# Hawkeye-FineGrained/Hawkeye

Hardware: NVIDIA H100
Metric: 448x448 images/sec, BCNN VGG-16 train step (fwd+CE+bwd+grad all-reduce+SGD), device-timed, max over ranks (higher is better)
Workload: dtype tf32 (fp32 storage, fp32 accumulate)

## Files before the change

### hawkeye_b200/csrc/conv.cu

```cuda
#include <stdlib.h>

#include "common.cuh"
#include "host.h"
#include "gemm.h"
#include "../../include/hawkeye_b200.h"

namespace hk {

__global__ void pack_weights_kernel(const float* __restrict__ W, float* __restrict__ Wf, float* __restrict__ Wd,
                                    int Cout, int Cin, int round) {
  const size_t n = (size_t)Cout * Cin * 9;
  for (size_t i = blockIdx.x * (size_t)blockDim.x + threadIdx.x; i < n; i += (size_t)gridDim.x * blockDim.x) {
    const int t = i % 9;
    const int ci = (i / 9) % Cin;
    const int co = i / ((size_t)9 * Cin);
    const float v = round ? tf32_round(W[i]) : W[i];
    if (Wf) Wf[((size_t)t * Cout + co) * Cin + ci] = v;
    if (Wd) Wd[((size_t)(8 - t) * Cin + ci) * Cout + co] = v;
  }
}
__global__ void unpack_wgrad_kernel(const float* __restrict__ dWp, float* __restrict__ dW, int Cout, int Cin, int accumulate) {
  const size_t n = (size_t)Cout * Cin * 9;
  for (size_t i = blockIdx.x * (size_t)blockDim.x + threadIdx.x; i < n; i += (size_t)gridDim.x * blockDim.x) {
    const int t = i % 9;
    const int ci = (i / 9) % Cin;
    const int co = i / ((size_t)9 * Cin);
    const float v = dWp[((size_t)t * Cin + ci) * Cout + co];
    dW[i] = accumulate ? dW[i] + v : v;
  }
}

struct ConvArgs {
  float* Y;
  const float* bias;
  const float* mask;
  int N, H, W, Cin, Cout;
  int TW, TH, TN;
  int tiles_w, tiles_h, tiles_n;
  int relu;
  int stride;
  const float* addend;
  int no_round;
  float* P;
  unsigned char* code;
  int pool_nchw;
};

__device__ __forceinline__ void epi_pool_store(const ConvArgs& a, const float* v, int TW, int w, int h, int n, int co,
                                               bool valid) {
  const bool writer = valid && !(w & 1) && !(h & 1);
  const int Ho = a.H >> 1, Wo = a.W >> 1;
  const size_t pp = ((size_t)n * Ho + (h >> 1)) * Wo + (w >> 1);
  float m[32];
  unsigned char cd[32];
#pragma unroll
  for (int j = 0; j < 32; ++j) {
    const float v0 = v[j];
    const float v1 = __shfl_xor_sync(0xffffffffu, v0, 1);
    const float v2 = __shfl_xor_sync(0xffffffffu, v0, TW);
    const float v3 = __shfl_xor_sync(0xffffffffu, v0, TW | 1);
    float mm = v0;
    unsigned char k = 0;
    if (v1 > mm) { mm = v1; k = 1; }
    if (v2 > mm) { mm = v2; k = 2; }
    if (v3 > mm) { mm = v3; k = 3; }
    m[j] = mm;
    cd[j] = k | (mm > 0.f ? 4 : 0);
  }
  if (!writer) return;
  if (a.code) {
    uint32_t pk[8];
#pragma unroll
    for (int j = 0; j < 8; ++j)
      pk[j] = (uint32_t)cd[4 * j] | ((uint32_t)cd[4 * j + 1] << 8) | ((uint32_t)cd[4 * j + 2] << 16) | ((uint32_t)cd[4 * j + 3] << 24);
    uint4* cp = reinterpret_cast<uint4*>(a.code + pp * a.Cout + co);
    cp[0] = make_uint4(pk[0], pk[1], pk[2], pk[3]);
    cp[1] = make_uint4(pk[4], pk[5], pk[6], pk[7]);
  }
  if (!a.pool_nchw) {
    float4* dst = reinterpret_cast<float4*>(a.P + pp * a.Cout + co);
#pragma unroll
    for (int j = 0; j < 8; ++j) dst[j] = make_float4(m[4 * j], m[4 * j + 1], m[4 * j + 2], m[4 * j + 3]);
  } else {
    const size_t hw = (size_t)Ho * Wo;
    float* dst = a.P + ((size_t)n * a.Cout + co) * hw + (size_t)(h >> 1) * Wo + (w >> 1);
#pragma unroll
    for (int j = 0; j < 32; ++j) dst[(size_t)j * hw] = m[j];
  }
}

constexpr int CONV_THREADS = 384;

template <int BN>
struct ConvCfg {
  static constexpr int STAGES = 4;
  static constexpr int A_BYTES = 128 * 128;
  static constexpr int B_BYTES = BN * 128;
  static constexpr int STAGE_BYTES = A_BYTES + B_BYTES;
  static constexpr int ACC_TILE = 2 * 128 * 33 * 4;
  static constexpr int SMEM = STAGES * STAGE_BYTES + 1024 + 256 + ACC_TILE;
};

template <bool POOLED = false>
__device__ __forceinline__ void epi_chunk(const ConvArgs& a, float (&v)[32], int w, int h, int n, size_t pix, int co,
                                          bool valid) {
  if (valid && co < a.Cout) {
    if (!POOLED && a.addend) {
      const float4* ad = reinterpret_cast<const float4*>(a.addend + pix * a.Cout + co);
#pragma unroll
      for (int j = 0; j < 8; ++j) {
        const float4 t = ad[j];
// ... 114 lines not shown
        const int tap = kb / nchunk, ck = kb - tap * nchunk;
        const int kh = tap / 3, kw = tap - kh * 3;
        mbar_wait(&empty[s], ph ^ 1);
        mbar_expect_tx(&full[s], Cfg::STAGE_BYTES);
        tma_load_4d(sA + s * Cfg::A_BYTES, &tmX, &full[s], ck * 32, w0 * a.stride + kw - 1, h0 * a.stride + kh - 1, n0);
        tma_load_3d(sB + s * Cfg::B_BYTES, &tmW, &full[s], ck * 32, co0, tap);
      }
    }
  } else {
    regs_alloc<224>();
    const int ct = threadIdx.x - 128;
    const int wg = ct >> 7;
    float acc[NACC];
    for (int kb = 0; kb < nk; ++kb) {
      const int s = kb % Cfg::STAGES;
      const uint32_t ph = (kb / Cfg::STAGES) & 1;
      mbar_wait(&full[s], ph);
      const uint64_t a_base = make_sdesc(smem_u32(sA + s * Cfg::A_BYTES + wg * 64 * 128));
      const uint64_t b_base = make_sdesc(smem_u32(sB + s * Cfg::B_BYTES));
      wgmma_fence();
#pragma unroll
      for (int ks = 0; ks < 4; ++ks) wgmma_tf32(acc, a_base + ks * 2, b_base + ks * 2, (kb | ks) != 0);
      wgmma_commit();
      wgmma_wait<1>();
      wgmma_keep(acc);
      if (kb > 0 && (ct & 127) == 0) mbar_arrive(&empty[(kb - 1) % Cfg::STAGES]);
    }
    wgmma_wait<0>();
    wgmma_keep(acc);
    conv_epilogue<BN>(a, acc, acc_tile, w0, h0, n0, co0, ct);
  }
}

static void pick_tile(int W, int H, int N, int target, int* TW, int* TH, int* TN) {
  int tw = 1;
  while (tw * 2 <= 16 && W % (tw * 2) == 0 && tw * 2 <= target) tw *= 2;
  int th = 1;
  while (th * 2 * tw <= target && H % (th * 2) == 0) th *= 2;
  int tn = target / (tw * th);
  *TW = tw; *TH = th; *TN = tn;
  (void)N;
}

static int make_act_map(CUtensorMap* tm, const float* X, int N, int H, int W, int C, int TW, int TH, int TN,
                        int stride = 1) {
  uint64_t dims[4] = {(uint64_t)C, (uint64_t)W, (uint64_t)H, (uint64_t)N};
  uint64_t strides[3] = {(uint64_t)C * 4, (uint64_t)W * C * 4, (uint64_t)H * W * C * 4};
  uint32_t box[4] = {32, (uint32_t)(TW * stride), (uint32_t)(TH * stride), (uint32_t)TN};
  uint32_t estr[4] = {1, (uint32_t)stride, (uint32_t)stride, 1};
  return make_tmap(tm, X, 4, dims, strides, box, stride > 1 ? estr : nullptr);
}

template <int BN>
static int launch_conv(const CUtensorMap& tmX, const CUtensorMap& tmW, const ConvArgs& a, cudaStream_t stream) {
  using Cfg = ConvCfg<BN>;
  if (int r = allow_dynamic_smem<conv3x3_igemm_kernel<BN>>(Cfg::SMEM, BN == 64 ? "conv<64>" : "conv<128>")) return r;
  dim3 grid(a.tiles_w * a.tiles_h * a.tiles_n, (a.Cout + BN - 1) / BN);
  conv3x3_igemm_kernel<BN><<<grid, CONV_THREADS, Cfg::SMEM, stream>>>(tmX, tmW, a);
  HK_LAUNCH_CHECK("conv3x3_igemm_kernel");
  return 0;
}

constexpr int CONV_V2_THREADS = 512;

enum { EPI_MAP = 0, EPI_UNPOOL = 1, EPI_FIRST_WGRAD = 2 };
constexpr int FW_HALO = 3 * 10 * 18;
constexpr int FW_HALO_BYTES = 2 * FW_HALO * 4;
struct FirstWgradArgs {
  const float* img;
  float* part;
};

__device__ __forceinline__ void mma_m16n8k8_tf32(float (&d)[4], const uint32_t (&a)[4], uint32_t b0, uint32_t b1) {
  asm volatile("mma.sync.aligned.m16n8k8.row.col.f32.tf32.tf32.f32 {%0, %1, %2, %3}, {%4, %5, %6, %7}, {%8, %9}, "
               "{%0, %1, %2, %3};\n"
               : "+f"(d[0]), "+f"(d[1]), "+f"(d[2]), "+f"(d[3])
               : "r"(a[0]), "r"(a[1]), "r"(a[2]), "r"(a[3]), "r"(b0), "r"(b1));
}

template <int BN, bool RESIDENT>
struct ConvV2Cfg {
  static constexpr int A_BYTES = 160 * 128;
  static constexpr int B_TILE = BN * 128;
  static constexpr int STAGE_BYTES = A_BYTES + (RESIDENT ? 0 : 3 * B_TILE);
  static constexpr int STAGES = RESIDENT ? 2 : (BN == 64 ? 3 : 2);
  static constexpr int WRES_BYTES = RESIDENT ? 18 * B_TILE : 0;
  static constexpr int PIECES = STAGES == 2 && !RESIDENT ? 3 : 1;
  static constexpr int STG_LD = BN + 8;
  static constexpr int STG_BYTES = 128 * STG_LD * 4;
  static constexpr int SMEM = STAGES * STAGE_BYTES + WRES_BYTES + 1024 + 256 + STG_BYTES;
};

template <int BN, bool RESIDENT, int TW, int EPI>
__global__ void __launch_bounds__(CONV_V2_THREADS, 1)
conv3x3_igemm_v2_kernel(const __grid_constant__ CUtensorMap tmX, const __grid_constant__ CUtensorMap tmW, ConvArgs a,
                        int n_ntiles, int total_tiles, FirstWgradArgs fw) {
  using Cfg = ConvV2Cfg<BN, RESIDENT>;
  static_assert(EPI != EPI_FIRST_WGRAD || (BN == 64 && RESIDENT && TW == 16), "conv1_1 weight gradient: 64 -> 64, 16 x 8");
  constexpr int NACC = BN / 2;
  constexpr int TN = 16 / TW;
  constexpr int WG_ROWS = TW == 16 ? 64 : 80;
  extern __shared__ uint8_t smem_raw[];
  uint8_t* smem = reinterpret_cast<uint8_t*>((reinterpret_cast<uintptr_t>(smem_raw) + 1023) & ~uintptr_t(1023));
  uint8_t* stages = smem;
  uint8_t* wres = smem + Cfg::STAGES * Cfg::STAGE_BYTES;
  uint64_t* full = reinterpret_cast<uint64_t*>(wres + Cfg::WRES_BYTES);
  uint64_t* empty = full + Cfg::STAGES * Cfg::PIECES;
  uint64_t* wbar = empty + Cfg::STAGES;
  uint64_t* stg_full = wbar + 1;
  uint64_t* stg_empty = wbar + 2;
  float* stg = reinterpret_cast<float*>(wres + Cfg::WRES_BYTES + 256);

  const int warp = threadIdx.x >> 5;
  const int nchunk = a.Cin / 32;
  const int nkb = nchunk * 3;

  if (threadIdx.x == 0) {
    tma_prefetch_desc(&tmX);
    tma_prefetch_desc(&tmW);
    for (int s = 0; s < Cfg::STAGES; ++s) mbar_init(&empty[s], 2);
    for (int i = 0; i < Cfg::STAGES * Cfg::PIECES; ++i) mbar_init(&full[i], 1);
    mbar_init(wbar, 1);
    mbar_init(stg_full, 256);
    mbar_init(stg_empty, 128);
    fence_barrier_init();
  }
  __syncthreads();

  if (warp >= 12 && EPI == EPI_MAP && a.P) {
    const int r = threadIdx.x - 384;
    int j = 0;
    for (int t = blockIdx.x; t < total_tiles; t += gridDim.x, ++j) {
      int pt = t / n_ntiles;
      const int co0 = (t - pt * n_ntiles) * BN;
      const int tw = pt % a.tiles_w; pt /= a.tiles_w;
      const int th = pt % a.tiles_h; pt /= a.tiles_h;
      mbar_wait(stg_full, j & 1);
      const int w = tw * TW + (r & (TW - 1)), h = th * 8 + ((r / TW) & 7), n = pt * TN + r / (TW * 8);
      const bool valid = TN == 1 || n < a.N;
      const size_t pix = ((size_t)n * a.H + h) * a.W + w;
#pragma unroll 1
      for (int c = 0; c < BN / 32; ++c) {
        float v[32];
        const float4* src = reinterpret_cast<const float4*>(stg + r * Cfg::STG_LD + c * 32);
#pragma unroll
        for (int k = 0; k < 8; ++k) {
          const float4 q = src[k];
          v[4 * k] = q.x; v[4 * k + 1] = q.y; v[4 * k + 2] = q.z; v[4 * k + 3] = q.w;
        }
        if (c == BN / 32 - 1) mbar_arrive(stg_empty);
        epi_chunk<true>(a, v, w, h, n, pix, co0 + c * 32, valid);
      }
    }
  } else if (warp >= 12) {
    const int e = threadIdx.x - 384;
    const int ew = e >> 5, sub = (e >> 3) & 3, u4 = (e & 7) * 4;
    const int p0 = ew * 32 + sub;
    const int eoff0 = (TW == 16 ? (p0 >> 4) * a.W + (p0 & 15) : ((p0 >> 6) * a.H + ((p0 >> 3) & 7)) * a.W + (p0 & 7)) * a.Cout + u4;
    const int erow = a.W * a.Cout, e4 = 4 * a.Cout;
    auto eoff = [&](int k) { return eoff0 + (k / (TW / 4)) * erow + (k % (TW / 4)) * e4; };
    const float* srow = stg + (ew * 32 + sub) * Cfg::STG_LD + u4;
    auto tile_org = [&](int t, size_t& org, int& co0) {
      co0 = (t % n_ntiles) * BN;
      int pt = t / n_ntiles;
      const int tw = pt % a.tiles_w; pt /= a.tiles_w;
      const int th = pt % a.tiles_h; pt /= a.tiles_h;
      org = (((size_t)pt * TN * a.H + th * 8) * a.W + tw * TW) * a.Cout;
      return pt * TN + (TW == 16 ? 0 : ew >> 1) < a.N;
    };
    auto tile_pos = [&](int t, int& tw, int& th, int& tn) {
      int pt = t / n_ntiles;
      tw = pt % a.tiles_w; pt /= a.tiles_w;
      th = pt % a.tiles_h; tn = pt / a.tiles_h;
    };
    const int frow = 2 * a.W * a.Cout;
    const int uoff0 = (TW == 16 ? 2 * (p0 >> 4) * frow + 2 * (p0 & 15) * a.Cout
                                : ((p0 >> 6) * 2 * a.H + 2 * ((p0 >> 3) & 7)) * frow + 2 * (p0 & 7) * a.Cout) + u4;
    auto uoff = [&](int k) { return uoff0 + (k / (TW / 4)) * 2 * frow + (k % (TW / 4)) * 8 * a.Cout; };
    float* halo = stg + 128 * Cfg::STG_LD;
    float dacc[4][4] = {};
    const int lane = e & 31, g = lane >> 2, tq = lane & 3;
    int hoff[4];
#pragma unroll
    for (int nt = 0; nt < 4; ++nt) {
      const int jj = 8 * nt + g;
      hoff[nt] = jj < 27 ? (jj / 9) * 180 + (jj % 9 / 3) * 18 + jj % 3 : 0;
    }
    int co0 = 0, j = 0;
    size_t org = 0;
    for (int t = blockIdx.x; t < total_tiles; t += gridDim.x, ++j) {
      const bool valid = tile_org(t, org, co0);
      if constexpr (EPI == EPI_FIRST_WGRAD) {
        int tw, th, tn;
        tile_pos(t, tw, th, tn);
        float* hb = halo + (j & 1) * FW_HALO;
        for (int i = e; i < FW_HALO; i += 128) {
          const int ci = i / 180, hh = th * 8 - 1 + i / 18 % 10, ww = tw * 16 - 1 + i % 18;
          hb[i] = hh >= 0 && hh < a.H && ww >= 0 && ww < a.W
                      ? tf32_round(__ldg(fw.img + (((size_t)tn * 3 + ci) * a.H + hh) * a.W + ww)) : 0.f;
        }
      }
      mbar_wait(stg_full, j & 1);
#pragma unroll
      for (int c = 0; c < BN / 32; ++c) {
// ... 21 lines not shown
#pragma unroll
            for (int k = 0; k < 8; ++k) mk[k] = __ldcs(reinterpret_cast<const float4*>(a.mask + org + co + eoff(k)));
#pragma unroll
            for (int k = 0; k < 8; ++k) {
              v[k].x = mk[k].x > 0.f ? v[k].x : 0.f; v[k].y = mk[k].y > 0.f ? v[k].y : 0.f;
              v[k].z = mk[k].z > 0.f ? v[k].z : 0.f; v[k].w = mk[k].w > 0.f ? v[k].w : 0.f;
            }
          }
          if constexpr (EPI == EPI_MAP) {
#pragma unroll
            for (int k = 0; k < 8; ++k)
              __stcs(reinterpret_cast<float4*>(a.Y + org + co + eoff(k)),
                     make_float4(tf32_round(v[k].x), tf32_round(v[k].y), tf32_round(v[k].z), tf32_round(v[k].w)));
          } else if constexpr (EPI == EPI_UNPOOL) {
            int tw, th, tn;
            tile_pos(t, tw, th, tn);
            float* dst = a.Y + (((size_t)tn * TN * 2 * a.H + th * 16) * 2 * a.W + tw * 2 * TW) * a.Cout + co;
            uint32_t cd[8];
#pragma unroll
            for (int k = 0; k < 8; ++k) cd[k] = __ldcs(reinterpret_cast<const unsigned int*>(a.code + org + co + eoff(k)));
#pragma unroll
            for (int k = 0; k < 8; ++k) {
              const float4 q = make_float4((cd[k] & 4u) ? tf32_round(v[k].x) : 0.f, (cd[k] & (4u << 8)) ? tf32_round(v[k].y) : 0.f,
                                           (cd[k] & (4u << 16)) ? tf32_round(v[k].z) : 0.f,
                                           (cd[k] & (4u << 24)) ? tf32_round(v[k].w) : 0.f);
              float* o = dst + uoff(k);
#pragma unroll
              for (int pos = 0; pos < 4; ++pos)
                __stcs(reinterpret_cast<float4*>(o + (pos >> 1) * frow + (pos & 1) * a.Cout),
                       make_float4((cd[k] & 3u) == (uint32_t)pos ? q.x : 0.f, (cd[k] >> 8 & 3u) == (uint32_t)pos ? q.y : 0.f,
                                   (cd[k] >> 16 & 3u) == (uint32_t)pos ? q.z : 0.f,
                                   (cd[k] >> 24 & 3u) == (uint32_t)pos ? q.w : 0.f));
            }
          } else {
#pragma unroll
            for (int k = 0; k < 8; ++k)
              *reinterpret_cast<float4*>(stg + (ew * 32 + sub + 4 * k) * Cfg::STG_LD + u4 + c * 32) =
                  make_float4(tf32_round(v[k].x), tf32_round(v[k].y), tf32_round(v[k].z), tf32_round(v[k].w));
          }
        }
      }
      if constexpr (EPI == EPI_FIRST_WGRAD) {
        named_bar(1, 128);
        const float* hb = halo + (j & 1) * FW_HALO;
        const float* arow = stg + tq * Cfg::STG_LD + 16 * ew + g;
#pragma unroll 4
        for (int ks = 0; ks < 16; ++ks) {
          const float* ap = arow + 8 * ks * Cfg::STG_LD;
          const uint32_t af[4] = {__float_as_uint(ap[0]), __float_as_uint(ap[8]), __float_as_uint(ap[4 * Cfg::STG_LD]),
                                  __float_as_uint(ap[4 * Cfg::STG_LD + 8])};
          const int hp = (ks >> 1) * 18 + 8 * (ks & 1) + tq;
#pragma unroll
          for (int nt = 0; nt < 4; ++nt) {
            float b0 = hb[hoff[nt] + hp], b1 = hb[hoff[nt] + hp + 4];
            if (nt == 3 && g >= 3) b0 = b1 = g == 3 ? 1.f : 0.f;
            mma_m16n8k8_tf32(dacc[nt], af, __float_as_uint(b0), __float_as_uint(b1));
          }
        }
        mbar_arrive(stg_empty);
      }
    }
    if constexpr (EPI == EPI_FIRST_WGRAD) {
      float* dst = fw.part + (size_t)blockIdx.x * 64 * 32;
#pragma unroll
      for (int nt = 0; nt < 4; ++nt)
#pragma unroll
        for (int i = 0; i < 4; ++i) dst[(16 * ew + g + 8 * (i >> 1)) * 32 + 8 * nt + 2 * tq + (i & 1)] = dacc[nt][i];
    }
  } else if (warp < 4) {
    if (threadIdx.x == 0) {
      if (RESIDENT) {
        mbar_expect_tx(wbar, Cfg::WRES_BYTES);
        for (int tap = 0; tap < 9; ++tap)
          for (int ck = 0; ck < 2; ++ck) tma_load_3d(wres + (tap * 2 + ck) * Cfg::B_TILE, &tmW, wbar, ck * 32, 0, tap);
      }
      int kbg = 0;
      for (int t = blockIdx.x; t < total_tiles; t += gridDim.x) {
        const int nt = t % n_ntiles;
        int pt = t / n_ntiles;
        const int tw = pt % a.tiles_w; pt /= a.tiles_w;
        const int th = pt % a.tiles_h; pt /= a.tiles_h;
        const int w0 = tw * TW, h0 = th * 8, n0 = pt * TN, co0 = nt * BN;
        for (int kb = 0; kb < nkb; ++kb, ++kbg) {
          const int s = kbg % Cfg::STAGES;
          const uint32_t ph = (kbg / Cfg::STAGES) & 1;
          const int ck = kb / 3, kw = kb - ck * 3;
          mbar_wait(&empty[s], ph ^ 1);
          uint64_t* f = full + s * Cfg::PIECES;
          uint8_t* st = stages + s * Cfg::STAGE_BYTES;
          mbar_expect_tx(&f[0], Cfg::PIECES == 3 ? Cfg::A_BYTES + Cfg::B_TILE : Cfg::STAGE_BYTES);
          tma_load_4d(st, &tmX, &f[0], ck * 32, w0 + kw - 1, h0 - 1, n0);
          if (!RESIDENT) {
#pragma unroll
            for (int kh = 0; kh < 3; ++kh) {
              uint64_t* fk = &f[Cfg::PIECES == 3 ? kh : 0];
              if (Cfg::PIECES == 3 && kh > 0) mbar_expect_tx(fk, Cfg::B_TILE);
              tma_load_3d(st + Cfg::A_BYTES + kh * Cfg::B_TILE, &tmW, fk, ck * 32, co0, kh * 3 + kw);
            }
          }
        }
      }
    }
  } else {
    const int ct = threadIdx.x - 128;
    const int wg = ct >> 7;
    if (RESIDENT) mbar_wait(wbar, 0);
    float acc[NACC];
#pragma unroll
    for (int i = 0; i < NACC; ++i) acc[i] = 0.f;
    float* frag = stg + (wg * 64 + ((ct >> 5) & 3) * 16 + ((ct & 31) >> 2)) * Cfg::STG_LD + 2 * (ct & 3);
    int kbg = 0, j = 0;
    for (int t = blockIdx.x; t < total_tiles; t += gridDim.x, ++j) {
      for (int kb = 0; kb < nkb; ++kb, ++kbg) {
        const int s = kbg % Cfg::STAGES;
        const int ck = kb / 3, kw = kb - ck * 3;
        const uint32_t ph = (kbg / Cfg::STAGES) & 1;
        const uint32_t a_addr = smem_u32(stages + s * Cfg::STAGE_BYTES) + wg * WG_ROWS * 128;
#pragma unroll
        for (int kh = 0; kh < 3; ++kh) {
          if (kh < Cfg::PIECES) {
            mbar_wait(&full[s * Cfg::PIECES + kh], ph);
            wgmma_fence();
          }
          const uint32_t b_addr = RESIDENT ? smem_u32(wres + ((kh * 3 + kw) * 2 + ck) * Cfg::B_TILE)
                                           : smem_u32(stages + s * Cfg::STAGE_BYTES + Cfg::A_BYTES + kh * Cfg::B_TILE);
          const uint64_t ad = make_sdesc(a_addr + kh * TW * 128), bd = make_sdesc(b_addr);
#pragma unroll
          for (int ks = 0; ks < 4; ++ks) wgmma_tf32(acc, ad + ks * 2, bd + ks * 2, (kb | kh | ks) != 0);
          if (kh >= 3 - Cfg::PIECES) wgmma_commit();
          if (kh == 3 - Cfg::PIECES) {
            wgmma_wait<1>();
            wgmma_keep(acc);
            if (kb > 0 && (ct & 127) == 0) mbar_arrive(&empty[(kbg - 1) % Cfg::STAGES]);
          }
        }
      }
      wgmma_wait<0>();
      wgmma_keep(acc);
      if ((ct & 127) == 0) mbar_arrive(&empty[(kbg - 1) % Cfg::STAGES]);
      mbar_wait(stg_empty, (j & 1) ^ 1);
#pragma unroll
      for (int i = 0; i < NACC / 4; ++i) {
        *reinterpret_cast<float2*>(frag + 8 * i) = make_float2(acc[4 * i], acc[4 * i + 1]);
        *reinterpret_cast<float2*>(frag + 8 * Cfg::STG_LD + 8 * i) = make_float2(acc[4 * i + 2], acc[4 * i + 3]);
      }
      mbar_arrive(stg_full);
    }
  }
}

template <int BN, bool RESIDENT, int TW, int EPI = EPI_MAP>
static int launch_conv_v2(const float* x, const float* wp, ConvArgs a, int N, int H, int W, cudaStream_t stream,
                          FirstWgradArgs fw = {}) {
  using Cfg = ConvV2Cfg<BN, RESIDENT>;
  constexpr int SMEM = Cfg::SMEM + (EPI == EPI_FIRST_WGRAD ? FW_HALO_BYTES : 0);
  static_assert(SMEM <= 232448, "conv_v2: dynamic shared memory above the sm_90 opt-in limit");
  if (int r = allow_dynamic_smem<conv3x3_igemm_v2_kernel<BN, RESIDENT, TW, EPI>>(SMEM, BN == 64 ? "conv_v2<64>" : "conv_v2<128>"))
    return r;
  a.TW = TW; a.TH = 8; a.TN = 16 / TW;
  a.tiles_w = W / TW; a.tiles_h = H / 8; a.tiles_n = (N + a.TN - 1) / a.TN;
  const int n_ntiles = (a.Cout + BN - 1) / BN;
  const long long total = (long long)a.tiles_w * a.tiles_h * a.tiles_n * n_ntiles;
  HK_REQUIRE(total < (1ll << 31), HK_ERR_UNSUPPORTED, "conv3x3: too many tiles");
  HK_REQUIRE((long long)H * W * a.Cout < (1ll << 30), HK_ERR_UNSUPPORTED, "conv3x3: map too large");
  CUtensorMap tmX, tmW;
  int r;
  {
    uint64_t dims[4] = {(uint64_t)a.Cin, (uint64_t)W, (uint64_t)H, (uint64_t)N};
    uint64_t strides[3] = {(uint64_t)a.Cin * 4, (uint64_t)W * a.Cin * 4, (uint64_t)H * W * a.Cin * 4};
    uint32_t box[4] = {32, (uint32_t)TW, 10, (uint32_t)a.TN};
    if ((r = make_tmap(&tmX, x, 4, dims, strides, box))) return r;
  }
  {
    uint64_t dims[3] = {(uint64_t)a.Cin, (uint64_t)a.Cout, 9};
    uint64_t strides[2] = {(uint64_t)a.Cin * 4, (uint64_t)a.Cin * a.Cout * 4};
    uint32_t box[3] = {32, (uint32_t)BN, 1};
    if ((r = make_tmap(&tmW, wp, 3, dims, strides, box))) return r;
  }
  const int sms = num_sms();
  const int grid = total < sms ? (int)total : sms;
  conv3x3_igemm_v2_kernel<BN, RESIDENT, TW, EPI><<<grid, CONV_V2_THREADS, SMEM, stream>>>(tmX, tmW, a, n_ntiles, (int)total, fw);
  HK_LAUNCH_CHECK("conv3x3_igemm_v2_kernel");
  return 0;
}

template <int TW, int EPI = EPI_MAP>
static int launch_conv_v2(const float* x, const float* wp, const ConvArgs& a, int N, int H, int W, cudaStream_t stream) {
  if (a.Cin == 64 && a.Cout == 64) return launch_conv_v2<64, true, TW, EPI>(x, wp, a, N, H, W, stream);
  if (a.Cout <= 64) return launch_conv_v2<64, false, TW, EPI>(x, wp, a, N, H, W, stream);
  return launch_conv_v2<128, false, TW, EPI>(x, wp, a, N, H, W, stream);
}

static int conv3x3_igemm_1x(const float* x, const float* wp, const float* bias, const float* mask, const float* addend,
                            float* y, int N, int H, int W, int Cin, int Cout, int relu, cudaStream_t stream, int stride,
                            int no_round, float* pooled = nullptr, unsigned char* code = nullptr,
                            int pool_nchw = 0);

int conv3x3_igemm(const float* x, const float* wp, const float* bias, const float* mask, float* y, int N, int H, int W,
                  int Cin, int Cout, int relu, cudaStream_t stream, int stride = 1) {
  if (!precise()) return conv3x3_igemm_1x(x, wp, bias, mask, nullptr, y, N, H, W, Cin, Cout, relu, stream, stride, 0);
  HK_REQUIRE(x && wp && y, HK_ERR_ARG, "conv3x3: null pointer");
  const size_t nx = (size_t)N * H * W * Cin, nw = (size_t)9 * Cout * Cin;
  Scratch sx(2 * nx * sizeof(float), stream), sw(2 * nw * sizeof(float), stream);
  HK_REQUIRE(sx.p && sw.p, HK_ERR_DRIVER, "conv3x3 (precise): cudaMallocAsync of the operand halves failed");
  float *xh = sx.f(), *xl = xh + nx, *wh = sw.f(), *wl = wh + nw;
  int r;
  if ((r = tf32_split(x, xh, xl, nx, stream))) return r;
  if ((r = tf32_split(wp, wh, wl, nw, stream))) return r;
  if ((r = conv3x3_igemm_1x(xh, wl, nullptr, nullptr, nullptr, y, N, H, W, Cin, Cout, 0, stream, stride, 1))) return r;
  if ((r = conv3x3_igemm_1x(xl, wh, nullptr, nullptr, y, y, N, H, W, Cin, Cout, 0, stream, stride, 1))) return r;
  return conv3x3_igemm_1x(xh, wh, bias, mask, y, y, N, H, W, Cin, Cout, relu, stream, stride, 1);
}

static int conv3x3_igemm_1x(const float* x, const float* wp, const float* bias, const float* mask, const float* addend,
                            float* y, int N, int H, int W, int Cin, int Cout, int relu, cudaStream_t stream, int stride,
                            int no_round, float* pooled, unsigned char* code, int pool_nchw) {
  const int Hin = H, Win = W;
  if (stride == 2) {
    HK_REQUIRE(H % 2 == 0 && W % 2 == 0, HK_ERR_UNSUPPORTED, "conv3x3 stride 2: even H/W required");
    H /= 2; W /= 2;
  }
  HK_REQUIRE(x && wp && (y || pooled), HK_ERR_ARG, "conv3x3: null pointer");
// ... 553 lines not shown
__global__ void maxpool2x2_fwd_idx_kernel(const float* __restrict__ x, float* __restrict__ y, unsigned char* __restrict__ code,
                                          int N, int H, int W, int C, int out_nchw) {
  const int Ho = H / 2, Wo = W / 2, C4 = C / 4;
  const size_t total = (size_t)N * Ho * Wo * C4;
  for (size_t i = blockIdx.x * (size_t)blockDim.x + threadIdx.x; i < total; i += (size_t)gridDim.x * blockDim.x) {
    const int c4 = i % C4;
    size_t p = i / C4;
    const int wo = p % Wo; p /= Wo;
    const int ho = p % Ho;
    const int n = p / Ho;
    const float4* base = reinterpret_cast<const float4*>(x + (((size_t)n * H + 2 * ho) * W + 2 * wo) * C) + c4;
    const float4 v0 = base[0], v1 = base[C4], v2 = base[(size_t)W * C4], v3 = base[(size_t)W * C4 + C4];
    float4 m = v0;
    uchar4 a = make_uchar4(0, 0, 0, 0);
#define HK_POOL_STEP(V, K)                     \
    if (V.x > m.x) { m.x = V.x; a.x = K; }     \
    if (V.y > m.y) { m.y = V.y; a.y = K; }     \
    if (V.z > m.z) { m.z = V.z; a.z = K; }     \
    if (V.w > m.w) { m.w = V.w; a.w = K; }
    HK_POOL_STEP(v1, 1) HK_POOL_STEP(v2, 2) HK_POOL_STEP(v3, 3)
#undef HK_POOL_STEP
    a.x |= m.x > 0.f ? 4 : 0; a.y |= m.y > 0.f ? 4 : 0; a.z |= m.z > 0.f ? 4 : 0; a.w |= m.w > 0.f ? 4 : 0;
    reinterpret_cast<uchar4*>(code)[i] = a;
    if (!out_nchw) {
      reinterpret_cast<float4*>(y + (((size_t)n * Ho + ho) * Wo + wo) * C)[c4] = m;
    } else {
      const size_t hw = (size_t)Ho * Wo, o = ((size_t)n * C + c4 * 4) * hw + (size_t)ho * Wo + wo;
      y[o] = m.x; y[o + hw] = m.y; y[o + 2 * hw] = m.z; y[o + 3 * hw] = m.w;
    }
  }
}
__global__ void maxpool2x2_bwd_idx_kernel(const unsigned char* __restrict__ code, const float* __restrict__ dy,
                                          float* __restrict__ dx, int N, int H, int W, int C, int dy_nchw) {
  const int Ho = H / 2, Wo = W / 2, C4 = C / 4;
  const size_t total = (size_t)N * Ho * Wo * C4;
  for (size_t i = blockIdx.x * (size_t)blockDim.x + threadIdx.x; i < total; i += (size_t)gridDim.x * blockDim.x) {
    const int c4 = i % C4;
    size_t p = i / C4;
    const int wo = p % Wo; p /= Wo;
    const int ho = p % Ho;
    const int n = p / Ho;
    const uchar4 a = reinterpret_cast<const uchar4*>(code)[i];
    float4 g;
    if (!dy_nchw) {
      g = reinterpret_cast<const float4*>(dy)[i];
    } else {
      const size_t hw = (size_t)Ho * Wo, o = ((size_t)n * C + c4 * 4) * hw + (size_t)ho * Wo + wo;
      g = make_float4(dy[o], dy[o + hw], dy[o + 2 * hw], dy[o + 3 * hw]);
    }
    g.x = (a.x & 4) ? g.x : 0.f; g.y = (a.y & 4) ? g.y : 0.f; g.z = (a.z & 4) ? g.z : 0.f; g.w = (a.w & 4) ? g.w : 0.f;
    float4* base = reinterpret_cast<float4*>(dx + (((size_t)n * H + 2 * ho) * W + 2 * wo) * C) + c4;
#define HK_POOL_OUT(K) make_float4((a.x & 3) == K ? g.x : 0.f, (a.y & 3) == K ? g.y : 0.f, (a.z & 3) == K ? g.z : 0.f, \
                                   (a.w & 3) == K ? g.w : 0.f)
    base[0] = HK_POOL_OUT(0);
    base[C4] = HK_POOL_OUT(1);
    base[(size_t)W * C4] = HK_POOL_OUT(2);
    base[(size_t)W * C4 + C4] = HK_POOL_OUT(3);
#undef HK_POOL_OUT
  }
}

__global__ void bias_grad_kernel(const float* __restrict__ dy, float* __restrict__ db, size_t npix, int C) {
  const int c = threadIdx.x % C;
  const int lanes_per_c = blockDim.x / C > 0 ? blockDim.x / C : 1;
  const int sub = threadIdx.x / C;
  if (sub >= lanes_per_c) return;
  const size_t per = (npix + gridDim.x - 1) / gridDim.x;
  const size_t p0 = blockIdx.x * per, p1 = (p0 + per < npix) ? p0 + per : npix;
  for (int cc = c; cc < C; cc += (blockDim.x < C ? blockDim.x : C)) {
    float s = 0.f;
    for (size_t p = p0 + sub; p < p1; p += lanes_per_c) s += dy[p * C + cc];
    atomicAdd(db + cc, s);
  }
}

}

using namespace hk;

extern "C" {

int hk_conv3x3_pack_weights(const float* w, float* w_fwd, float* w_dgrad, int Cout, int Cin, void* stream) {
  HK_REQUIRE(w && (w_fwd || w_dgrad), HK_ERR_ARG, "hk_conv3x3_pack_weights: null pointer");
  pack_weights_kernel<<<grid_1d((size_t)Cout * Cin * 9, 256), 256, 0, (cudaStream_t)stream>>>(w, w_fwd, w_dgrad, Cout, Cin,
                                                                                              precise() ? 0 : 1);
  HK_LAUNCH_CHECK("pack_weights_kernel");
  return 0;
}

int hk_conv3x3_fwd(const float* x, const float* w_packed, const float* bias, float* y, int N, int H, int W, int Cin,
                   int Cout, int relu, void* stream) {
  return conv3x3_igemm(x, w_packed, bias, nullptr, y, N, H, W, Cin, Cout, relu, (cudaStream_t)stream);
}

int hk_conv3x3_fwd_pool(const float* x, const float* w_packed, const float* bias, float* pooled, unsigned char* code, int N,
                        int H, int W, int Cin, int Cout, int out_nchw, void* stream) {
  HK_REQUIRE(!precise(), HK_ERR_UNSUPPORTED, "hk_conv3x3_fwd_pool: not available in 3xTF32 mode (use conv + pool)");
  HK_REQUIRE(pooled, HK_ERR_ARG, "hk_conv3x3_fwd_pool: null output");
  return conv3x3_igemm_1x(x, w_packed, bias, nullptr, nullptr, nullptr, N, H, W, Cin, Cout, 1, (cudaStream_t)stream, 1,
                          0, pooled, code, out_nchw);
}

int hk_conv3x3_s2_fwd(const float* x, const float* w_packed, const float* bias, float* y, int N, int H, int W, int Cin,
                      int Cout, int relu, void* stream) {
  return conv3x3_igemm(x, w_packed, bias, nullptr, y, N, H, W, Cin, Cout, relu, (cudaStream_t)stream, 2);
}

int hk_conv3x3_dgrad(const float* dy, const float* w_dgrad_packed, const float* relu_mask_act, float* dx, int N, int H,
                     int W, int Cin, int Cout, void* stream) {
  return conv3x3_igemm(dy, w_dgrad_packed, nullptr, relu_mask_act, dx, N, H, W, Cout, Cin, 0, (cudaStream_t)stream);
}

int hk_conv3x3_dgrad_unpool(const float* dy, const float* w_dgrad_packed, const unsigned char* code, float* dx_full, int N,
                            int H, int W, int Cin, int Cout, void* stream) {
  HK_REQUIRE(!precise(), HK_ERR_UNSUPPORTED, "hk_conv3x3_dgrad_unpool: not available in 3xTF32 mode");
  HK_REQUIRE(dy && w_dgrad_packed && code && dx_full, HK_ERR_ARG, "hk_conv3x3_dgrad_unpool: null pointer");
  HK_REQUIRE(N > 0 && H > 0 && W > 0, HK_ERR_ARG, "hk_conv3x3_dgrad_unpool: empty map");
  HK_REQUIRE(Cin % 32 == 0 && Cout % 32 == 0, HK_ERR_UNSUPPORTED,
             "hk_conv3x3_dgrad_unpool: Cin=%d Cout=%d must be multiples of 32", Cin, Cout);
  HK_REQUIRE(H % 8 == 0 && W % 8 == 0, HK_ERR_UNSUPPORTED, "hk_conv3x3_dgrad_unpool: %dx%d map is not a multiple of 8x8",
             H, W);
  HK_REQUIRE(4ll * H * W * Cin < (1ll << 31), HK_ERR_UNSUPPORTED, "hk_conv3x3_dgrad_unpool: map too large");
  HK_REQUIRE(aligned16(dy) && aligned16(w_dgrad_packed) && aligned16(code) && aligned16(dx_full), HK_ERR_ALIGN,
             "hk_conv3x3_dgrad_unpool: pointer not 16-byte aligned");
  ConvArgs a = {};
  a.Y = dx_full; a.code = const_cast<unsigned char*>(code);
  a.N = N; a.H = H; a.W = W; a.Cin = Cout; a.Cout = Cin; a.stride = 1;
  if (W % 16 == 0) return launch_conv_v2<16, EPI_UNPOOL>(dy, w_dgrad_packed, a, N, H, W, (cudaStream_t)stream);
  return launch_conv_v2<8, EPI_UNPOOL>(dy, w_dgrad_packed, a, N, H, W, (cudaStream_t)stream);
}

size_t hk_conv3x3_dgrad_first_wgrad_workspace_bytes(void) { return (size_t)num_sms() * 64 * 32 * sizeof(float); }

int hk_conv3x3_dgrad_first_wgrad_acc(const float* dy, const float* w_dgrad_packed, const float* relu_mask_act,
                                     const float* x_nchw, float* dw1, float* db1, int N, int H, int W, int Cin, int Cout,
                                     void* workspace, size_t workspace_bytes, int accumulate, void* stream_) {
  cudaStream_t stream = (cudaStream_t)stream_;
  HK_REQUIRE(!precise(), HK_ERR_UNSUPPORTED, "hk_conv3x3_dgrad_first_wgrad: not available in 3xTF32 mode");
  HK_REQUIRE(dy && w_dgrad_packed && x_nchw && dw1, HK_ERR_ARG, "hk_conv3x3_dgrad_first_wgrad: null pointer");
  HK_REQUIRE(N > 0 && H > 0 && W > 0, HK_ERR_ARG, "hk_conv3x3_dgrad_first_wgrad: empty map");
  HK_REQUIRE(Cin == 64 && Cout == 64, HK_ERR_UNSUPPORTED, "hk_conv3x3_dgrad_first_wgrad: Cin=%d Cout=%d (64 -> 64 only)",
             Cin, Cout);
  HK_REQUIRE(W % 16 == 0 && H % 8 == 0, HK_ERR_UNSUPPORTED,
             "hk_conv3x3_dgrad_first_wgrad: %dx%d map is not tiled by 16x8", H, W);
  HK_REQUIRE(aligned16(dy) && aligned16(w_dgrad_packed) && (!relu_mask_act || aligned16(relu_mask_act)), HK_ERR_ALIGN,
             "hk_conv3x3_dgrad_first_wgrad: pointer not 16-byte aligned");
  HK_REQUIRE(workspace && workspace_bytes >= hk_conv3x3_dgrad_first_wgrad_workspace_bytes(), HK_ERR_WORKSPACE,
             "hk_conv3x3_dgrad_first_wgrad: workspace too small");
  const long long tiles = (long long)(W / 16) * (H / 8) * N;
  HK_REQUIRE(tiles < (1ll << 31), HK_ERR_UNSUPPORTED, "hk_conv3x3_dgrad_first_wgrad: too many tiles");
  float* part = static_cast<float*>(workspace);
  ConvArgs a = {};
  a.mask = relu_mask_act;
  a.N = N; a.H = H; a.W = W; a.Cin = Cout; a.Cout = Cin; a.stride = 1;
  int r = launch_conv_v2<64, true, 16, EPI_FIRST_WGRAD>(dy, w_dgrad_packed, a, N, H, W, stream, FirstWgradArgs{x_nchw, part});
  if (r) return r;
  const int G = tiles < num_sms() ? (int)tiles : num_sms();
  if ((r = sum_splits(part, G, 64 * 32, 64, 27, 32, dw1, 27, nullptr, accumulate, stream))) return r;
  if (!db1) return 0;
  return sum_splits(part + 27, G, 64 * 32, 64, 1, 32, db1, 1, nullptr, accumulate, stream);
}

size_t hk_conv3x3_wgrad_workspace_bytes(int Cin, int Cout) { return (size_t)9 * Cin * Cout * sizeof(float); }

int hk_conv3x3_wgrad_acc(const float* x, const float* dy, float* dw, float* db, int N, int H, int W, int Cin, int Cout,
                         void* workspace, size_t workspace_bytes, int accumulate, void* stream_) {
  cudaStream_t stream = (cudaStream_t)stream_;
  HK_REQUIRE(workspace && workspace_bytes >= hk_conv3x3_wgrad_workspace_bytes(Cin, Cout), HK_ERR_WORKSPACE,
             "hk_conv3x3_wgrad: workspace too small");
  HK_REQUIRE(dw, HK_ERR_ARG, "hk_conv3x3_wgrad: null dw");
  float* dwp = static_cast<float*>(workspace);
  int r = conv3x3_wgrad(x, dy, dwp, db, N, H, W, Cin, Cout, stream, !accumulate);
  if (r) return r;
  unpack_wgrad_kernel<<<grid_1d((size_t)Cout * Cin * 9, 256), 256, 0, stream>>>(dwp, dw, Cout, Cin, accumulate ? 1 : 0);
  HK_LAUNCH_CHECK("unpack_wgrad_kernel");
  return 0;
}

int hk_conv3x3_wgrad(const float* x, const float* dy, float* dw, float* db, int N, int H, int W, int Cin, int Cout,
                     void* workspace, size_t workspace_bytes, void* stream_) {
  return hk_conv3x3_wgrad_acc(x, dy, dw, db, N, H, W, Cin, Cout, workspace, workspace_bytes, 0, stream_);
}

size_t hk_conv3x3_first_fwd_workspace_bytes(int N, int H, int W, int Cout) {
  return ((size_t)N * H * W * 32 + (size_t)Cout * 32) * sizeof(float);
}

int hk_conv3x3_first_fwd(const float* x_nchw, const float* w, const float* bias, float* y_nhwc, int N, int H, int W,
                         int Cout, void* workspace, size_t workspace_bytes, void* stream_) {
  cudaStream_t stream = (cudaStream_t)stream_;
  HK_REQUIRE(x_nchw && w && y_nhwc, HK_ERR_ARG, "hk_conv3x3_first_fwd: null pointer");
  HK_REQUIRE(Cout % 4 == 0 && Cout <= 256, HK_ERR_UNSUPPORTED, "hk_conv3x3_first_fwd: Cout=%d unsupported", Cout);
  HK_REQUIRE(workspace && workspace_bytes >= hk_conv3x3_first_fwd_workspace_bytes(N, H, W, Cout), HK_ERR_WORKSPACE,
             "hk_conv3x3_first_fwd: workspace too small");
  const long long P = (long long)N * H * W;
  HK_REQUIRE(P < (1ll << 31), HK_ERR_UNSUPPORTED, "hk_conv3x3_first_fwd: too many pixels");
  float* x27 = static_cast<float*>(workspace);
  float* w27 = x27 + (size_t)P * 32;
  const int round = precise() ? 0 : 1;
  im2col_first_kernel<<<grid_1d((size_t)P, 128), 128, 0, stream>>>(x_nchw, x27, N, H, W, round);
  HK_LAUNCH_CHECK("im2col_first_kernel");
  pack_first_weights_kernel<<<(Cout * 32 + 127) / 128, 128, 0, stream>>>(w, bias, w27, Cout, round);
  HK_LAUNCH_CHECK("pack_first_weights_kernel");
  GemmEpi e = {};
  e.C = y_nhwc; e.ldc = Cout; e.alpha = 1.f;
  e.relu = 3;
  return gemm_tf32(x27, 0, 32, 0, w27, 0, 32, 0, e, (int)P, Cout, 32, 1, stream);
}

static int first_wgrad_splits(long long P) {
  for (int S = 592; S > 1; --S)
    if (P % S == 0) return S;
  return 1;
}

size_t hk_conv3x3_first_wgrad_workspace_bytes(int N, int H, int W, int Cout) {
  return (size_t)first_wgrad_splits((long long)N * H * W) * Cout * 32 * sizeof(float);
}

int hk_conv3x3_first_wgrad_acc(const float* x27, const float* dy_nhwc, float* dw, float* db, int N, int H, int W, int Cout,
                               void* workspace, size_t workspace_bytes, int accumulate, void* stream_);
int hk_conv3x3_first_wgrad(const float* x27, const float* dy_nhwc, float* dw, float* db, int N, int H, int W,
                           int Cout, void* workspace, size_t workspace_bytes, void* stream_) {
  return hk_conv3x3_first_wgrad_acc(x27, dy_nhwc, dw, db, N, H, W, Cout, workspace, workspace_bytes, 0, stream_);
}
int hk_conv3x3_first_wgrad_acc(const float* x27, const float* dy_nhwc, float* dw, float* db, int N, int H, int W, int Cout,
                               void* workspace, size_t workspace_bytes, int accumulate, void* stream_) {
  cudaStream_t stream = (cudaStream_t)stream_;
  HK_REQUIRE(x27 && dy_nhwc && dw, HK_ERR_ARG, "hk_conv3x3_first_wgrad: null pointer");
  HK_REQUIRE(Cout % 4 == 0 && Cout <= 128, HK_ERR_UNSUPPORTED, "hk_conv3x3_first_wgrad: Cout=%d unsupported", Cout);
  HK_REQUIRE(workspace && workspace_bytes >= hk_conv3x3_first_wgrad_workspace_bytes(N, H, W, Cout), HK_ERR_WORKSPACE,
             "hk_conv3x3_first_wgrad: workspace too small");
  const long long P = (long long)N * H * W;
  const int S = first_wgrad_splits(P);
  float* part = static_cast<float*>(workspace);
  int r = gemm_splitk(dy_nhwc, 1, Cout, x27, 1, 32, Cout, 32, P, S, part, dw, 27, 27, nullptr, accumulate, stream);
  if (r || !db) return r;
  return sum_splits(part + 27, S, (long long)Cout * 32, Cout, 1, 32, db, 1, nullptr, accumulate, stream);
}

int hk_conv3x3_first_fwd_direct(const float* x_nchw, const float* w, const float* bias, float* y_nhwc, int N, int H, int W,
                                int Cout, void* stream) {
  HK_REQUIRE(!precise(), HK_ERR_UNSUPPORTED, "hk_conv3x3_first_fwd_direct: not available in 3xTF32 mode");
  HK_REQUIRE(x_nchw && w && y_nhwc, HK_ERR_ARG, "hk_conv3x3_first_fwd_direct: null pointer");
  HK_REQUIRE(Cout == 64, HK_ERR_UNSUPPORTED, "hk_conv3x3_first_fwd_direct: Cout=%d unsupported (64 only)", Cout);
  HK_REQUIRE(N > 0 && H > 0 && W > 0, HK_ERR_ARG, "hk_conv3x3_first_fwd_direct: empty map");
  HK_REQUIRE((reinterpret_cast<uintptr_t>(y_nhwc) & 7) == 0, HK_ERR_ALIGN, "hk_conv3x3_first_fwd_direct: y not 8-byte aligned");
  const long long P = (long long)N * H * W;
  HK_REQUIRE(P < (1ll << 31), HK_ERR_UNSUPPORTED, "hk_conv3x3_first_fwd_direct: too many pixels");
  first_fwd_direct_kernel<<<(int)((P + FIRST_FWD_PIX - 1) / FIRST_FWD_PIX), 128, FIRST_FWD_SMEM, (cudaStream_t)stream>>>(
      x_nchw, w, bias, y_nhwc, N, H, W);
  HK_LAUNCH_CHECK("first_fwd_direct_kernel");
  return 0;
}

static int first_wgrad_direct_ctas() { return 2 * num_sms(); }

// ... 64 lines not shown
```

Before: 830.7.

## Decouple activation and weight rings in conv pipeline; tile weight pack/unpack transposes

For BN=128 non-resident conv tiles, the single stage buffer is split into a 3-slot activation ring and a 6-slot per-tap weight ring with separate barriers. Consumers release each weight slot one wgmma group late, so TMA loads can overlap compute at finer granularity. Other configs move to 4 stages with one barrier per stage. Separately, the weight pack and wgrad unpack kernels become shared-memory tiled transposes with coalesced global access; the finer barrier protocol is harder to verify and the larger ring costs shared memory.

Measured after the change: 845.6, median of 6. 1.02x the previous value.

```diff
diff --git a/hawkeye_b200/csrc/conv.cu b/hawkeye_b200/csrc/conv.cu
--- a/hawkeye_b200/csrc/conv.cu
+++ b/hawkeye_b200/csrc/conv.cu
@@ -7,26 +7,70 @@
 
 namespace hk {
 
-__global__ void pack_weights_kernel(const float* __restrict__ W, float* __restrict__ Wf, float* __restrict__ Wd,
-                                    int Cout, int Cin, int round) {
-  const size_t n = (size_t)Cout * Cin * 9;
-  for (size_t i = blockIdx.x * (size_t)blockDim.x + threadIdx.x; i < n; i += (size_t)gridDim.x * blockDim.x) {
-    const int t = i % 9;
-    const int ci = (i / 9) % Cin;
-    const int co = i / ((size_t)9 * Cin);
-    const float v = round ? tf32_round(W[i]) : W[i];
-    if (Wf) Wf[((size_t)t * Cout + co) * Cin + ci] = v;
-    if (Wd) Wd[((size_t)(8 - t) * Cin + ci) * Cout + co] = v;
-  }
-}
-__global__ void unpack_wgrad_kernel(const float* __restrict__ dWp, float* __restrict__ dW, int Cout, int Cin, int accumulate) {
-  const size_t n = (size_t)Cout * Cin * 9;
-  for (size_t i = blockIdx.x * (size_t)blockDim.x + threadIdx.x; i < n; i += (size_t)gridDim.x * blockDim.x) {
-    const int t = i % 9;
-    const int ci = (i / 9) % Cin;
-    const int co = i / ((size_t)9 * Cin);
-    const float v = dWp[((size_t)t * Cin + ci) * Cout + co];
-    dW[i] = accumulate ? dW[i] + v : v;
+constexpr int PACK_T = 32;
+constexpr int PACK_LD = PACK_T * 9 + 1;
+constexpr int PACK_THREADS = 256;
+constexpr int PACK_PER_THREAD = PACK_T * PACK_T * 9 / PACK_THREADS;
+
+__global__ void __launch_bounds__(PACK_THREADS)
+pack_weights_kernel(const float* __restrict__ W, float* __restrict__ Wf, float* __restrict__ Wd, int Cout, int Cin,
+                    int round) {
+  __shared__ float tile[PACK_T * PACK_LD];
+  const int ci0 = blockIdx.x * PACK_T, co0 = blockIdx.y * PACK_T;
+  const int nci = min(PACK_T, Cin - ci0), nco = min(PACK_T, Cout - co0);
+  float v[PACK_PER_THREAD];
+#pragma unroll
+  for (int k = 0; k < PACK_PER_THREAD; ++k) {
+    const int i = threadIdx.x + k * PACK_THREADS, co = i / (PACK_T * 9), r = i - co * (PACK_T * 9);
+    v[k] = co < nco && r < nci * 9 ? W[((size_t)(co0 + co) * Cin + ci0) * 9 + r] : 0.f;
+  }
+#pragma unroll
+  for (int k = 0; k < PACK_PER_THREAD; ++k) {
+    const int i = threadIdx.x + k * PACK_THREADS, co = i / (PACK_T * 9), r = i - co * (PACK_T * 9);
+    tile[co * PACK_LD + r] = round ? tf32_round(v[k]) : v[k];
+  }
+  __syncthreads();
+#pragma unroll 4
+  for (int k = 0; k < PACK_PER_THREAD; ++k) {
+    const int i = threadIdx.x + k * PACK_THREADS;
+    const int t = i / (PACK_T * PACK_T), a = (i / PACK_T) % PACK_T, b = i % PACK_T;
+    if (Wf && a < nco && b < nci) Wf[((size_t)t * Cout + co0 + a) * Cin + ci0 + b] = tile[a * PACK_LD + b * 9 + t];
+    if (Wd && a < nci && b < nco)
+      Wd[((size_t)(8 - t) * Cin + ci0 + a) * Cout + co0 + b] = tile[b * PACK_LD + a * 9 + t];
+  }
+}
+__global__ void __launch_bounds__(PACK_THREADS)
+unpack_wgrad_kernel(const float* __restrict__ dWp, float* __restrict__ dW, int Cout, int Cin, int accumulate) {
+  __shared__ float tile[PACK_T * PACK_LD];
+  const int ci0 = blockIdx.x * PACK_T, co0 = blockIdx.y * PACK_T;
+  const int nci = min(PACK_T, Cin - ci0), nco = min(PACK_T, Cout - co0);
+  float v[PACK_PER_THREAD];
+#pragma unroll
+  for (int k = 0; k < PACK_PER_THREAD; ++k) {
+    const int i = threadIdx.x + k * PACK_THREADS;
+    const int t = i / (PACK_T * PACK_T), ci = (i / PACK_T) % PACK_T, co = i % PACK_T;
+    v[k] = ci < nci && co < nco ? dWp[((size_t)t * Cin + ci0 + ci) * Cout + co0 + co] : 0.f;
+  }
+#pragma unroll
+  for (int k = 0; k < PACK_PER_THREAD; ++k) {
+    const int i = threadIdx.x + k * PACK_THREADS;
+    const int t = i / (PACK_T * PACK_T), ci = (i / PACK_T) % PACK_T, co = i % PACK_T;
+    tile[co * PACK_LD + ci * 9 + t] = v[k];
+  }
+  __syncthreads();
+  float* out = dW + ((size_t)co0 * Cin + ci0) * 9;
+  if (accumulate) {
+#pragma unroll
+    for (int k = 0; k < PACK_PER_THREAD; ++k) {
+      const int i = threadIdx.x + k * PACK_THREADS, co = i / (PACK_T * 9), r = i - co * (PACK_T * 9);
+      v[k] = co < nco && r < nci * 9 ? out[(size_t)co * Cin * 9 + r] : 0.f;
+    }
+  }
+#pragma unroll
+  for (int k = 0; k < PACK_PER_THREAD; ++k) {
+    const int i = threadIdx.x + k * PACK_THREADS, co = i / (PACK_T * 9), r = i - co * (PACK_T * 9);
+    const float g = tile[co * PACK_LD + r];
+    if (co < nco && r < nci * 9) out[(size_t)co * Cin * 9 + r] = accumulate ? v[k] + g : g;
   }
 }
 
@@ -307,13 +351,19 @@
 struct ConvV2Cfg {
   static constexpr int A_BYTES = 160 * 128;
   static constexpr int B_TILE = BN * 128;
+  static constexpr bool SPLIT = BN == 128 && !RESIDENT;
+  static constexpr int NH = 3, NW = 6;
+  static_assert(NW == 2 * 3, "step k uses weight slots 3 (k & 1) + kh");
+  static constexpr int LAG = 1;
   static constexpr int STAGE_BYTES = A_BYTES + (RESIDENT ? 0 : 3 * B_TILE);
-  static constexpr int STAGES = RESIDENT ? 2 : (BN == 64 ? 3 : 2);
+  static constexpr int STAGES = RESIDENT ? 2 : 4;
+  static constexpr int RING_BYTES = SPLIT ? NH * A_BYTES + NW * B_TILE : STAGES * STAGE_BYTES;
+  static constexpr int NBAR = SPLIT ? NH + NW : STAGES;
   static constexpr int WRES_BYTES = RESIDENT ? 18 * B_TILE : 0;
-  static constexpr int PIECES = STAGES == 2 && !RESIDENT ? 3 : 1;
   static constexpr int STG_LD = BN + 8;
   static constexpr int STG_BYTES = 128 * STG_LD * 4;
-  static constexpr int SMEM = STAGES * STAGE_BYTES + WRES_BYTES + 1024 + 256 + STG_BYTES;
+  static constexpr int SMEM = RING_BYTES + WRES_BYTES + 1024 + 256 + STG_BYTES;
+  static_assert(2 * NBAR + 3 <= 32, "barriers beyond their 256 bytes");
 };
 
 template <int BN, bool RESIDENT, int TW, int EPI>
@@ -328,10 +378,11 @@
   extern __shared__ uint8_t smem_raw[];
   uint8_t* smem = reinterpret_cast<uint8_t*>((reinterpret_cast<uintptr_t>(smem_raw) + 1023) & ~uintptr_t(1023));
   uint8_t* stages = smem;
-  uint8_t* wres = smem + Cfg::STAGES * Cfg::STAGE_BYTES;
+  uint8_t* wring = smem + Cfg::NH * Cfg::A_BYTES;
+  uint8_t* wres = smem + Cfg::RING_BYTES;
   uint64_t* full = reinterpret_cast<uint64_t*>(wres + Cfg::WRES_BYTES);
-  uint64_t* empty = full + Cfg::STAGES * Cfg::PIECES;
-  uint64_t* wbar = empty + Cfg::STAGES;
+  uint64_t* empty = full + Cfg::NBAR;
+  uint64_t* wbar = empty + Cfg::NBAR;
   uint64_t* stg_full = wbar + 1;
   uint64_t* stg_empty = wbar + 2;
   float* stg = reinterpret_cast<float*>(wres + Cfg::WRES_BYTES + 256);
@@ -343,8 +394,10 @@
   if (threadIdx.x == 0) {
     tma_prefetch_desc(&tmX);
     tma_prefetch_desc(&tmW);
-    for (int s = 0; s < Cfg::STAGES; ++s) mbar_init(&empty[s], 2);
-    for (int i = 0; i < Cfg::STAGES * Cfg::PIECES; ++i) mbar_init(&full[i], 1);
+    for (int i = 0; i < Cfg::NBAR; ++i) {
+      mbar_init(&full[i], 1);
+      mbar_init(&empty[i], 2);
+    }
     mbar_init(wbar, 1);
     mbar_init(stg_full, 256);
     mbar_init(stg_empty, 128);
@@ -532,20 +585,31 @@
         const int th = pt % a.tiles_h; pt /= a.tiles_h;
         const int w0 = tw * TW, h0 = th * 8, n0 = pt * TN, co0 = nt * BN;
         for (int kb = 0; kb < nkb; ++kb, ++kbg) {
-          const int s = kbg % Cfg::STAGES;
-          const uint32_t ph = (kbg / Cfg::STAGES) & 1;
           const int ck = kb / 3, kw = kb - ck * 3;
-          mbar_wait(&empty[s], ph ^ 1);
-          uint64_t* f = full + s * Cfg::PIECES;
-          uint8_t* st = stages + s * Cfg::STAGE_BYTES;
-          mbar_expect_tx(&f[0], Cfg::PIECES == 3 ? Cfg::A_BYTES + Cfg::B_TILE : Cfg::STAGE_BYTES);
-          tma_load_4d(st, &tmX, &f[0], ck * 32, w0 + kw - 1, h0 - 1, n0);
-          if (!RESIDENT) {
+          if constexpr (Cfg::SPLIT) {
+            const int hs = kbg % Cfg::NH;
+            mbar_wait(&empty[hs], ((kbg / Cfg::NH) & 1) ^ 1);
+            mbar_expect_tx(&full[hs], Cfg::A_BYTES);
+            tma_load_4d(stages + hs * Cfg::A_BYTES, &tmX, &full[hs], ck * 32, w0 + kw - 1, h0 - 1, n0);
+            const int wb = 3 * (kbg & 1);
 #pragma unroll
             for (int kh = 0; kh < 3; ++kh) {
-              uint64_t* fk = &f[Cfg::PIECES == 3 ? kh : 0];
-              if (Cfg::PIECES == 3 && kh > 0) mbar_expect_tx(fk, Cfg::B_TILE);
-              tma_load_3d(st + Cfg::A_BYTES + kh * Cfg::B_TILE, &tmW, fk, ck * 32, co0, kh * 3 + kw);
+              uint64_t* fb = &full[Cfg::NH + wb + kh];
+              mbar_wait(&empty[Cfg::NH + wb + kh], ((kbg >> 1) & 1) ^ 1);
+              mbar_expect_tx(fb, Cfg::B_TILE);
+              tma_load_3d(wring + (wb + kh) * Cfg::B_TILE, &tmW, fb, ck * 32, co0, kh * 3 + kw);
+            }
+          } else {
+            const int s = kbg % Cfg::STAGES;
+            const uint32_t ph = (kbg / Cfg::STAGES) & 1;
+            mbar_wait(&empty[s], ph ^ 1);
+            uint8_t* st = stages + s * Cfg::STAGE_BYTES;
+            mbar_expect_tx(&full[s], Cfg::STAGE_BYTES);
+            tma_load_4d(st, &tmX, &full[s], ck * 32, w0 + kw - 1, h0 - 1, n0);
+            if (!RESIDENT) {
+#pragma unroll
+              for (int kh = 0; kh < 3; ++kh)
+                tma_load_3d(st + Cfg::A_BYTES + kh * Cfg::B_TILE, &tmW, &full[s], ck * 32, co0, kh * 3 + kw);
             }
           }
         }
@@ -560,34 +624,67 @@
     for (int i = 0; i < NACC; ++i) acc[i] = 0.f;
     float* frag = stg + (wg * 64 + ((ct >> 5) & 3) * 16 + ((ct & 31) >> 2)) * Cfg::STG_LD + 2 * (ct & 3);
     int kbg = 0, j = 0;
+    int hs = 0;
+    uint32_t hph = 0;
     for (int t = blockIdx.x; t < total_tiles; t += gridDim.x, ++j) {
       for (int kb = 0; kb < nkb; ++kb, ++kbg) {
-        const int s = kbg % Cfg::STAGES;
         const int ck = kb / 3, kw = kb - ck * 3;
-        const uint32_t ph = (kbg / Cfg::STAGES) & 1;
-        const uint32_t a_addr = smem_u32(stages + s * Cfg::STAGE_BYTES) + wg * WG_ROWS * 128;
-#pragma unroll
-        for (int kh = 0; kh < 3; ++kh) {
-          if (kh < Cfg::PIECES) {
-            mbar_wait(&full[s * Cfg::PIECES + kh], ph);
+        if constexpr (Cfg::SPLIT) {
+          const uint32_t a_addr = smem_u32(stages + hs * Cfg::A_BYTES) + wg * WG_ROWS * 128;
+          const int wb = 3 * (kbg & 1);
+          const uint32_t wph = (kbg >> 1) & 1;
+#pragma unroll
+          for (int kh = 0; kh < 3; ++kh) {
+            if (kh == 0) mbar_wait(&full[hs], hph);
+            mbar_wait(&full[Cfg::NH + wb + kh], wph);
             wgmma_fence();
+            const uint64_t ad = make_sdesc(a_addr + kh * TW * 128);
+            const uint64_t bd = make_sdesc(smem_u32(wring + (wb + kh) * Cfg::B_TILE));
+#pragma unroll
+            for (int ks = 0; ks < 4; ++ks) wgmma_tf32(acc, ad + ks * 2, bd + ks * 2, (kb | kh | ks) != 0);
+            wgmma_commit();
+            wgmma_wait<Cfg::LAG>();
+            wgmma_keep(acc);
+            const int rkh = (kh + 3 - Cfg::LAG) % 3;
+            const bool prev = kh < Cfg::LAG;
+            if ((kb > 0 || !prev) && (ct & 127) == 0) {
+              mbar_arrive(&empty[Cfg::NH + (prev ? 3 - wb : wb) + rkh]);
+              if (rkh == 2) mbar_arrive(&empty[prev ? (hs == 0 ? Cfg::NH - 1 : hs - 1) : hs]);
+            }
           }
-          const uint32_t b_addr = RESIDENT ? smem_u32(wres + ((kh * 3 + kw) * 2 + ck) * Cfg::B_TILE)
-                                           : smem_u32(stages + s * Cfg::STAGE_BYTES + Cfg::A_BYTES + kh * Cfg::B_TILE);
-          const uint64_t ad = make_sdesc(a_addr + kh * TW * 128), bd = make_sdesc(b_addr);
-#pragma unroll
-          for (int ks = 0; ks < 4; ++ks) wgmma_tf32(acc, ad + ks * 2, bd + ks * 2, (kb | kh | ks) != 0);
-          if (kh >= 3 - Cfg::PIECES) wgmma_commit();
-          if (kh == 3 - Cfg::PIECES) {
-            wgmma_wait<1>();
-            wgmma_keep(acc);
-            if (kb > 0 && (ct & 127) == 0) mbar_arrive(&empty[(kbg - 1) % Cfg::STAGES]);
+          if (++hs == Cfg::NH) { hs = 0; hph ^= 1; }
+        } else {
+          const int s = kbg % Cfg::STAGES;
+          const uint32_t ph = (kbg / Cfg::STAGES) & 1;
+          const uint32_t a_addr = smem_u32(stages + s * Cfg::STAGE_BYTES) + wg * WG_ROWS * 128;
+          mbar_wait(&full[s], ph);
+          wgmma_fence();
+#pragma unroll
+          for (int kh = 0; kh < 3; ++kh) {
+            const uint32_t b_addr = RESIDENT ? smem_u32(wres + ((kh * 3 + kw) * 2 + ck) * Cfg::B_TILE)
+                                             : smem_u32(stages + s * Cfg::STAGE_BYTES + Cfg::A_BYTES + kh * Cfg::B_TILE);
+            const uint64_t ad = make_sdesc(a_addr + kh * TW * 128), bd = make_sdesc(b_addr);
+#pragma unroll
+            for (int ks = 0; ks < 4; ++ks) wgmma_tf32(acc, ad + ks * 2, bd + ks * 2, (kb | kh | ks) != 0);
           }
+          wgmma_commit();
+          wgmma_wait<1>();
+          wgmma_keep(acc);
+          if (kb > 0 && (ct & 127) == 0) mbar_arrive(&empty[(kbg - 1) % Cfg::STAGES]);
         }
       }
       wgmma_wait<0>();
       wgmma_keep(acc);
-      if ((ct & 127) == 0) mbar_arrive(&empty[(kbg - 1) % Cfg::STAGES]);
+      if ((ct & 127) == 0) {
+        if constexpr (Cfg::SPLIT) {
+          const int wb = 3 * ((kbg - 1) & 1);
+#pragma unroll
+          for (int kh = 3 - Cfg::LAG; kh < 3; ++kh) mbar_arrive(&empty[Cfg::NH + wb + kh]);
+          mbar_arrive(&empty[hs == 0 ? Cfg::NH - 1 : hs - 1]);
+        } else {
+          mbar_arrive(&empty[(kbg - 1) % Cfg::STAGES]);
+        }
+      }
       mbar_wait(stg_empty, (j & 1) ^ 1);
 #pragma unroll
       for (int i = 0; i < NACC / 4; ++i) {
@@ -1307,8 +1404,9 @@
 
 int hk_conv3x3_pack_weights(const float* w, float* w_fwd, float* w_dgrad, int Cout, int Cin, void* stream) {
   HK_REQUIRE(w && (w_fwd || w_dgrad), HK_ERR_ARG, "hk_conv3x3_pack_weights: null pointer");
-  pack_weights_kernel<<<grid_1d((size_t)Cout * Cin * 9, 256), 256, 0, (cudaStream_t)stream>>>(w, w_fwd, w_dgrad, Cout, Cin,
-                                                                                              precise() ? 0 : 1);
+  if (Cout <= 0 || Cin <= 0) return 0;
+  pack_weights_kernel<<<dim3((Cin + PACK_T - 1) / PACK_T, (Cout + PACK_T - 1) / PACK_T), PACK_THREADS, 0,
+                        (cudaStream_t)stream>>>(w, w_fwd, w_dgrad, Cout, Cin, precise() ? 0 : 1);
   HK_LAUNCH_CHECK("pack_weights_kernel");
   return 0;
 }
@@ -1397,7 +1495,8 @@
   float* dwp = static_cast<float*>(workspace);
   int r = conv3x3_wgrad(x, dy, dwp, db, N, H, W, Cin, Cout, stream, !accumulate);
   if (r) return r;
-  unpack_wgrad_kernel<<<grid_1d((size_t)Cout * Cin * 9, 256), 256, 0, stream>>>(dwp, dw, Cout, Cin, accumulate ? 1 : 0);
+  unpack_wgrad_kernel<<<dim3((Cin + PACK_T - 1) / PACK_T, (Cout + PACK_T - 1) / PACK_T), PACK_THREADS, 0, stream>>>(
+      dwp, dw, Cout, Cin, accumulate ? 1 : 0);
   HK_LAUNCH_CHECK("unpack_wgrad_kernel");
   return 0;
 }
```
